# opherlieber/rltime

Measured on AMD Instinct MI355X. Metric: sampled transitions/sec (= learner steps/sec x B x T), IQN-LSTM B=512 T=80 84x84x4, higher is better.
Workload: dtype f32

## Files before the change

### include/mirl.h

```cpp
#ifndef MIRL_H
#define MIRL_H

#include <stdint.h>

#ifdef __cplusplus
extern "C" {
#endif

#define MIRL_OK 0
#define MIRL_NEED_MORE 1
#define MIRL_ERR_ARG (-1)
#define MIRL_ERR_HIP (-2)
#define MIRL_ERR_STATE (-3)
#define MIRL_ERR_NOGPU (-4)

#define MIRL_MODE_UNIFORM 0
#define MIRL_MODE_PER 1

typedef struct mirl_replay mirl_replay;

typedef struct mirl_replay_config {
  int64_t size;
  int32_t num_envs;
  int32_t env_base;
// ... 158 lines not shown
                       int32_t first, void* stream);

int mirl_frames_to_f32_nhwc(int64_t N, int32_t C, int32_t HW, const uint8_t* src, float scale,
                            float* dst, void* stream);
int mirl_frames_to_f32_nhwc_ex(int64_t N, int32_t C, int32_t HW, const uint8_t* src, float scale,
                               float* dst, int32_t per_wg, int32_t flags, void* stream);

int mirl_conv1_u8_supported(int32_t C, int32_t H, int32_t W, int32_t F, int32_t K, int32_t S);
int mirl_conv1_u8_wpk_floats(int64_t* out);
int mirl_conv1_bf16_set(int32_t mode);
int mirl_conv1_wrw_bf16_set(int32_t mode);
int mirl_conv1_u8_fwd(int64_t N, int32_t H, int32_t W, const uint8_t* x, const float* weight,
                      int64_t ws_o, int64_t ws_c, int64_t ws_h, int64_t ws_w, const float* bias,
                      float scale, float* wpk, float* y, void* stream);
int mirl_conv1_u8_fwd_ex(int64_t N, int32_t H, int32_t W, const uint8_t* x, const float* weight,
                         int64_t ws_o, int64_t ws_c, int64_t ws_h, int64_t ws_w, const float* bias,
                         float scale, float* wpk, float* y, int32_t flags, void* stream);

int mirl_conv1_u8_wrw_scratch_floats(int64_t* out);
int mirl_conv1_u8_wrw(int64_t N, int32_t H, int32_t W, const uint8_t* x, const float* g, float scale,
                      float* scratch, float* dw, int64_t ws_o, int64_t ws_c, int64_t ws_h, int64_t ws_w,
                      void* stream);
int mirl_conv1_u8_wrw_ex(int64_t N, int32_t H, int32_t W, const uint8_t* x, const float* g, float scale,
                         float* scratch, float* dw, int64_t ws_o, int64_t ws_c, int64_t ws_h, int64_t ws_w,
                         int32_t flags, void* stream);
int mirl_conv1_u8_wrw_masked(int64_t N, int32_t H, int32_t W, const uint8_t* x, const float* dy, const float* y, float scale,
                             float* scratch, float* dw, int64_t ws_o, int64_t ws_c, int64_t ws_h, int64_t ws_w,
                             float* db, void* stream);

int mirl_conv2_bwd_data_supported(int32_t C, int32_t F, int32_t K, int32_t S, int32_t IH, int32_t IW,
                                  int32_t OH, int32_t OW);
int mirl_conv2_bwd_data(int64_t N, int32_t OH, int32_t OW, const float* g, const float* weight,
                        int64_t ws_o, int64_t ws_c, int64_t ws_h, int64_t ws_w, float* wpk, float* dx,
                        void* stream);
int mirl_conv2_bwd_data_wpk_floats(int64_t* floats);
int mirl_conv2_bwd_data_ex(int64_t N, int32_t OH, int32_t OW, const float* g, const float* weight, int64_t ws_o,
                           int64_t ws_c, int64_t ws_h, int64_t ws_w, float* wpk, int64_t wpk_floats, float* dx, int32_t pipe,
                           void* stream);
int mirl_conv3_bwd_data_supported(int32_t C, int32_t F, int32_t K, int32_t S, int32_t IH, int32_t IW, int32_t OH, int32_t OW);
int mirl_conv3_bwd_data_wpk_floats(int64_t* floats);
int mirl_conv3_bwd_data(int64_t N, int32_t OH, int32_t OW, const float* g, const float* weight, int64_t ws_o,
                        int64_t ws_c, int64_t ws_h, int64_t ws_w, float* wpk, int64_t wpk_floats, float* dx, void* stream);

int mirl_gemm3_supported(int32_t layout, int64_t M, int64_t N, int64_t K);
int mirl_gemm3_workspace_bytes(int32_t layout, int64_t M, int64_t N, int64_t K, int64_t* bytes);
int mirl_gemm3(int32_t layout, int64_t M, int64_t N, int64_t K, const float* A, int64_t lda,
               const float* B, int64_t ldb, float* C, int64_t ldc, const float* bias, int32_t relu,
               void* workspace, int64_t workspace_bytes, void* stream);
int mirl_gemm3_mid_set(int32_t mode);
int mirl_gemm3_nt_mul(int64_t M, int64_t N, int64_t K, const float* A, int64_t lda, const float* B,
                      int64_t ldb, float* C, int64_t ldc, const float* bias, int32_t relu,
                      const float* mul, int64_t ldmul, int32_t group_shift, float* pre, int64_t ldpre,
                      void* stream);
int mirl_gemm3_head_workspace_bytes(int64_t M, int64_t N, int64_t* bytes);
int mirl_gemm3_nt_head(int64_t M, int64_t N, int64_t K, const float* A, int64_t lda, const float* B, int64_t ldb,
                       float* C, int64_t ldc, const float* bias, int32_t relu, const float* w2, int32_t O,
                       const float* bias2, float* out2, int64_t ldo, void* workspace, int64_t workspace_bytes, void* stream);
int mirl_gemm3_nn_qp_partial_rows(int64_t M, int64_t* rows);
int mirl_gemm3_nn_qp(int64_t M, int64_t N, int64_t K, const float* A, int64_t lda, const float* B, int64_t ldb,
                     const float* emb, int64_t ldemb, const float* x, int64_t ldx, float* d_pre, int64_t ldd,
                     float* dx, int64_t lddx, float* db_partial, void* stream);

int mirl_conv3_fwd_supported(int32_t C, int32_t F, int32_t KH, int32_t KW, int32_t S, int32_t H, int32_t W);
int mirl_conv3_fwd(int64_t N, int32_t H, int32_t W, int32_t C, int32_t F, int32_t KH, int32_t KW, int32_t S,
                   const float* x, const float* w, const float* bias, int32_t relu, float* y, void* stream);

int mirl_conv_wrw_b3_supported(int32_t C, int32_t F, int32_t KH, int32_t KW, int32_t S, int32_t H, int32_t W);
int mirl_conv_wrw_b3_scratch_bytes(int32_t C, int32_t F, int32_t KH, int32_t KW, int64_t* bytes);
int mirl_conv_wrw_b3(int64_t N, int32_t H, int32_t W, int32_t C, int32_t F, int32_t KH, int32_t KW, int32_t S,
                     const float* x, const float* g, void* scratch, int64_t scratch_bytes, float* dw, void* stream);

int mirl_bias_relu_rows(int64_t rows, int32_t C, float* y, const float* bias, void* stream);
int mirl_colsum_blocks(int64_t rows, int32_t C, int32_t* blocks);
int mirl_relu_bwd_bias_rows(int64_t rows, int32_t C, const float* dy, const float* y, float* g,
                            float* db, float* partial, int32_t blocks, void* stream);
int mirl_cos_embed(int64_t rows, int32_t D, const float* tau, const float* freq, float* phi, void* stream);
int mirl_cos_embed_rng(int64_t rows, int32_t D, uint64_t seed, const uint64_t* step, const float* freq,
                       float* phi, float* tau_out, void* stream);
int mirl_iqn_mul_fwd(int64_t M, int32_t N, int32_t C, const float* x, const float* emb, float* out, void* stream);
int mirl_iqn_mul_bwd(int64_t M, int32_t N, int32_t C, const float* g, const float* emb, const float* x,
                     float* d_pre, float* dx, float* db, float* partial, int32_t blocks, void* stream);

int mirl_dueling_tail_bwd(int64_t M, int32_t H1, int32_t Hv, int32_t A, int32_t Q, const float* ga,
                          const float* gv, const float* wo, const float* wq, const float* both,
                          float* g, float* db, float* partial, int32_t blocks, void* stream);
int mirl_dueling_tail_bwd_w(int64_t M, int32_t H1, int32_t Hv, int32_t A, int32_t Q, const float* ga,
                            const float* gv, const float* wo, const float* wq, const float* both, float* g,
                            float* db, float* partial, int32_t blocks, float* dwj, float* partial_w,
                            void* stream);

int mirl_actor_head(int32_t E, int32_t N, int32_t A, const float* adv, const float* val, int32_t Q,
                    const double* eps, const double* expo, double eps_min, const float* u, const int64_t* rnd,
                    int32_t* actions, float* qvalues, float* eps_used, void* stream);
int mirl_actor_head_rng(int32_t E, int32_t N, int32_t A, const float* adv, int32_t adv_pitch, const float* val, int32_t Q,
                        const double* eps, const double* expo, double eps_min, uint64_t rng_seed,
                        const uint64_t* rng_step, int32_t* actions, float* qvalues, float* eps_used, void* stream);
int mirl_actor_head_c51(int32_t E, int32_t A, int32_t Z, const float* adv, int32_t adv_pitch, const float* val,
                        int32_t val_pitch, const float* support, const double* eps, const double* expo, double eps_min,
                        const float* u, const int64_t* rnd, uint64_t rng_seed, const uint64_t* rng_step,
                        int32_t* actions, float* qvalues, float* eps_used, void* stream);
int mirl_stack_shift(int32_t E, int32_t P, int32_t plane_bytes, const uint8_t* in, uint8_t* out,
                     const uint8_t* newest, const uint8_t* dones, void* stream);
#define MIRL_STEP_ADVANCE (~0ull)
int mirl_actor_pre(int32_t E, int32_t H, int32_t A, const float* rewards_raw, const uint8_t* dones,
                   const int32_t* actions, const float* h, const float* c, float* xh_tail, int64_t xh_pitch,
                   float* c_in, float* state_pack, float* initials, float* rewards_out, uint8_t* dones_out,
// ... 92 lines not shown
```

### rltime_amd/_lib.py

```python
import ctypes as C
import os

import torch

_HERE = os.path.dirname(os.path.abspath(__file__))
LIB_PATH = os.path.join(_HERE, "librltime_hip.so")

MIRL_OK = 0
MIRL_NEED_MORE = 1
MODE_UNIFORM = 0
MODE_PER = 1
INT32_MIN = -2 ** 31


MIRL_OK, MIRL_ERR_ARG, MIRL_ERR_HIP, MIRL_ERR_STATE, MIRL_ERR_NOGPU = 0, -1, -2, -3, -4


class MirlError(RuntimeError):
    code = None


class ReplayConfig(C.Structure):
    _fields_ = [
        ("size", C.c_int64),
# ... 75 lines not shown

_vp, _i32, _i64, _u64, _f64 = C.c_void_p, C.c_int32, C.c_int64, C.c_uint64, C.c_double
_P = C.POINTER

_SIGNATURES = {
    "mirl_device_count": [],
    "mirl_replay_create": [_P(ReplayConfig), _P(_vp)],
    "mirl_replay_destroy": [_vp],
    "mirl_replay_ingest": [_vp, _P(Ingest), _vp],
    "mirl_replay_ingest_plan": [_vp, _i32, _i32, _vp, _vp],
    "mirl_replay_ingest_planned": [_vp, _i32, _P(Ingest), _vp],
    "mirl_ingest_fused_set": [_i32],
    "mirl_replay_prime_stack": [_vp, _vp, _i64, _vp],
    "mirl_replay_needed_feed_count": [_vp, _i32, _i32, _P(_i64)],
    "mirl_replay_sample": [_vp, _i32, _f64, _vp, _u64, _vp, _vp, _vp, _vp, _vp, _vp, _vp],
    "mirl_replay_sample_ready": [_vp, _i32, _P(_i32)],
    "mirl_replay_sample_skip": [_vp, _i32],
    "mirl_replay_tree_root": [_vp, _vp, _vp],
    "mirl_replay_sample_global": [_vp, _i32, _i32, _i32, _i32, _i32, _vp, _f64, _u64, _vp, _vp, _vp, _vp, _vp, _vp, _vp, _vp],
    "mirl_replay_profile": [_vp, _i32, _P(_i64), _P(_f64)],
    "mirl_profile_set": [_i32],
    "mirl_profile_collect": [_P(_i32)],
    "mirl_profile_get": [_i32, C.c_char_p, _i32, _P(_i64), _P(_f64), _P(_f64)],
    "mirl_profile_get_flop": [_i32, _vp],
    "mirl_profile_reset": [],
    "mirl_replay_save": [_vp, C.c_char_p],
    "mirl_replay_load": [_vp, C.c_char_p],
    "mirl_replay_uniform_total": [_vp, _P(_i64)],
    "mirl_replay_set_train_quota": [_vp, _i64],
    "mirl_replay_state_rows": [_vp, _P(_i32), _P(_i32)],
    "mirl_replay_gather": [_vp, _i32, _vp, _vp, _vp, _vp, _P(Batch), _vp],
    "mirl_replay_update_losses": [_vp, _i64, _vp, _vp, _vp],
    "mirl_replay_stats": [_vp, _P(_i64), _P(_i64), _P(_i64), _P(_i64), _P(_i64)],
    "mirl_replay_env_meta": [_vp, _vp, _vp],
    "mirl_replay_free_slots": [_vp, _vp, _P(_i64)],
    "mirl_replay_slot_table": [_vp, _vp, _vp],
    "mirl_replay_tree_nodes": [_vp, _vp, _vp, _vp],
    "mirl_replay_tree_set_leaves": [_vp, _i64, _vp, _vp, _vp],
    "mirl_replay_tree_find": [_vp, _i32, _vp, _vp, _vp],
    "mirl_replay_losses_peek": [_vp, _i32, _i64, _i32, _vp],
    "mirl_q_target_dqn": [_i64, _i32, _vp, _vp, _vp, _vp, _vp, _f64, _f64, _vp, _vp],
    "mirl_q_target_iqn": [_i64, _i32, _i32, _i32, _vp, _vp, _vp, _vp, _vp, _f64, _f64, _vp, _vp],
    "mirl_loss_dqn": [_i64, _i32, _vp, _vp, _vp, _vp, _f64, _i32, _f64, _vp, _vp, _vp, _vp],
    "mirl_loss_iqn": [_i64, _i32, _i32, _i32, _vp, _vp, _vp, _vp, _vp, _f64, _f64, _vp, _vp, _vp, _vp],
    "mirl_q_target_c51": [_i64, _i32, _i32, _vp, _vp, _vp, _vp, _vp, _vp, _f64, _f64, _f64, _f64, _i32, _vp, _vp],
    "mirl_loss_c51": [_i64, _i32, _i32, _vp, _vp, _vp, _vp, _i32, _f64, _f64, _vp, _vp, _vp, _vp],
    "mirl_actor_head_c51": [_i32, _i32, _i32, _vp, _i32, _vp, _i32, _vp, _vp, _vp, _f64, _vp, _vp, _u64, _vp, _vp, _vp, _vp, _vp],
    "mirl_lstm_cell_fwd": [_i32, _i32, _vp, _vp, _vp, _vp, _vp, _vp, _vp, _vp],
    "mirl_lstm_seq_supported": [_i32, _i32, _i32],
    "mirl_lstm_seq_workspace_bytes": [_i32, _i32, _P(_i64)],
    "mirl_lstm_seq_fwd": [_i32, _i32, _i32, _vp, _vp, _vp, _vp, _vp, _vp, _vp, _vp, _vp, _vp, _vp, _i32, _vp, _vp],
    "mirl_lstm_seq_status": [_P(_i32)],
    "mirl_gemm3_mid_set": [_i32],
    "mirl_lstm_seq_fwd_grid": [_i32, _i32, _P(_i32), _P(_i64), _P(_i32), _P(_i32)],
    "mirl_lstm_seq_bwd_supported": [_i32, _i32, _i32],
    "mirl_lstm_seq_bwd_workspace_bytes": [_i32, _i32, _P(_i64)],
    "mirl_lstm_seq_bwd": [_i32, _i32, _i32, _vp, _vp, _vp, _vp, _vp, _vp, _vp, _vp],
    "mirl_lstm_cell_bwd": [_i32, _i32, _vp, _vp, _vp, _vp, _vp, _vp, _vp, _i32, _vp],
    "mirl_frames_to_f32_nhwc": [_i64, _i32, _i32, _vp, C.c_float, _vp, _vp],
    "mirl_frames_to_f32_nhwc_ex": [_i64, _i32, _i32, _vp, C.c_float, _vp, _i32, _i32, _vp],
    "mirl_conv1_u8_supported": [_i32, _i32, _i32, _i32, _i32, _i32],
    "mirl_conv1_bf16_set": [_i32],
    "mirl_conv1_wrw_bf16_set": [_i32],
    "mirl_conv1_u8_wpk_floats": [_P(_i64)],
    "mirl_conv1_u8_fwd": [_i64, _i32, _i32, _vp, _vp, _i64, _i64, _i64, _i64, _vp, C.c_float, _vp, _vp, _vp],
    "mirl_conv1_u8_fwd_ex": [_i64, _i32, _i32, _vp, _vp, _i64, _i64, _i64, _i64, _vp, C.c_float, _vp, _vp, _i32, _vp],
    "mirl_conv1_u8_wrw_scratch_floats": [_P(_i64)],
    "mirl_conv1_u8_wrw_ex": [_i64, _i32, _i32, _vp, _vp, C.c_float, _vp, _vp, _i64, _i64, _i64, _i64, _i32, _vp],
    "mirl_conv1_u8_wrw_masked": [_i64, _i32, _i32, _vp, _vp, _vp, C.c_float, _vp, _vp, _i64, _i64, _i64, _i64, _vp, _vp],
    "mirl_conv1_u8_wrw": [_i64, _i32, _i32, _vp, _vp, C.c_float, _vp, _vp, _i64, _i64, _i64, _i64, _vp],
    "mirl_conv2_bwd_data_supported": [_i32, _i32, _i32, _i32, _i32, _i32, _i32, _i32],
    "mirl_conv2_bwd_data": [_i64, _i32, _i32, _vp, _vp, _i64, _i64, _i64, _i64, _vp, _vp, _vp],
    "mirl_conv2_bwd_data_wpk_floats": [_P(_i64)],
    "mirl_conv3_bwd_data_supported": [_i32, _i32, _i32, _i32, _i32, _i32, _i32, _i32],
    "mirl_conv3_bwd_data_wpk_floats": [_P(_i64)],
    "mirl_conv3_bwd_data": [_i64, _i32, _i32, _vp, _vp, _i64, _i64, _i64, _i64, _vp, _i64, _vp, _vp],
    "mirl_conv2_bwd_data_ex": [_i64, _i32, _i32, _vp, _vp, _i64, _i64, _i64, _i64, _vp, _i64, _vp, _i32, _vp],
    "mirl_conv3_fwd_supported": [_i32, _i32, _i32, _i32, _i32, _i32, _i32],
    "mirl_conv3_fwd": [_i64, _i32, _i32, _i32, _i32, _i32, _i32, _i32, _vp, _vp, _vp, _i32, _vp, _vp],
    "mirl_conv_wrw_b3_supported": [_i32, _i32, _i32, _i32, _i32, _i32, _i32],
    "mirl_conv_wrw_b3_scratch_bytes": [_i32, _i32, _i32, _i32, _P(_i64)],
    "mirl_conv_wrw_b3": [_i64, _i32, _i32, _i32, _i32, _i32, _i32, _i32, _vp, _vp, _vp, _i64, _vp, _vp],
    "mirl_gemm3_supported": [_i32, _i64, _i64, _i64],
    "mirl_gemm3_workspace_bytes": [_i32, _i64, _i64, _i64, _P(_i64)],
    "mirl_gemm3": [_i32, _i64, _i64, _i64, _vp, _i64, _vp, _i64, _vp, _i64, _vp, _i32, _vp, _i64, _vp],
    "mirl_gemm3_nt_mul": [_i64, _i64, _i64, _vp, _i64, _vp, _i64, _vp, _i64, _vp, _i32, _vp, _i64, _i32, _vp, _i64, _vp],
    "mirl_gemm3_nn_qp_partial_rows": [_i64, _P(_i64)],
    "mirl_gemm3_nn_qp": [_i64, _i64, _i64, _vp, _i64, _vp, _i64, _vp, _i64, _vp, _i64, _vp, _i64, _vp, _i64, _vp, _vp],
    "mirl_gemm3_head_workspace_bytes": [_i64, _i64, _P(_i64)],
    "mirl_gemm3_nt_head": [_i64, _i64, _i64, _vp, _i64, _vp, _i64, _vp, _i64, _vp, _i32, _vp, _i32, _vp, _vp, _i64, _vp, _i64, _vp],
    "mirl_act_conv_supported": [_i32, _i32, _i32, _i32, _i32, _i32, _i32],
    "mirl_act_conv_fwd": [_i32, _i64, _i32, _i32, _vp, _vp, _vp, _vp, _i64, _vp],
    "mirl_act_lstm_supported": [_i32, _i32, _i32],
    "mirl_act_lstm_workspace_bytes": [_i32, _i32, _i32, _P(_i64)],
    "mirl_act_lstm_fwd": [_i32, _i32, _i32, _vp, _i64, _vp, _vp, _vp, _vp, _vp, _vp, _vp],
    "mirl_act_embed": [_i32, _i32, _i32, _i32, _vp, _vp, _vp, _u64, _vp, _vp, _vp, _vp, _vp, _vp],
    "mirl_act_head_supported": [_i32, _i32, _i32, _i32, _i32, _i32],
    "mirl_act_head_parts": [_i32, _i32, _P(_i32), _P(_i32)],
    "mirl_act_head_hidden": [_i32, _i32, _i32, _i32, _vp, _vp, _vp, _vp, _vp, _vp],
    "mirl_act_head_select": [_i32, _i32, _i32, _i32, _i32, _vp, _vp, _i32, _vp, _vp, _f64, _u64, _vp, _vp, _vp, _vp],
    "mirl_bias_relu_rows": [_i64, _i32, _vp, _vp, _vp],
    "mirl_colsum_blocks": [_i64, _i32, _P(_i32)],
    "mirl_relu_bwd_bias_rows": [_i64, _i32, _vp, _vp, _vp, _vp, _vp, _i32, _vp],
    "mirl_cos_embed": [_i64, _i32, _vp, _vp, _vp, _vp],
    "mirl_cos_embed_rng": [_i64, _i32, _u64, _vp, _vp, _vp, _vp, _vp],
    "mirl_adam_clip_workspace_bytes": [_i32, _vp, _vp],
# ... 95 lines not shown
```

### rltime_amd/csrc/gemm3.hip

```cpp
#include "common.hpp"
#include "split3.hpp"
#include <stdlib.h>

namespace mirl {

struct G3Args {
  const float* A; const float* B; float* C; const float* bias;
  int64_t M, N, K;
  int64_t lda, ldb, ldc;
  int relu;
  int mt, nt;
  int splits;
  int steps_per_split;
  const float* mul; int64_t ldmul; int mul_shift;
  float* pre; int64_t ldpre;
  int vec_ok;
  const float* w2; float* part;
  float* gsum; int64_t ldgsum;
};


template <bool KC>
struct G3Loader {
  const float* p[2];
  int64_t step;
  int64_t ld;
  int lds_off;
  __device__ __forceinline__ void init(const float* base, int64_t ld_, int64_t row0, int64_t rows, int64_t k0, int t) {
    ld = ld_;
    if (KC) {
      const int r = t >> 2, kq = t & 3;
#pragma unroll
      for (int h = 0; h < 2; ++h) {
        int64_t row = row0 + r + 128 * h; if (row > rows - 1) row = rows - 1;
        p[h] = base + row * ld + k0 + kq * 4;
      }
      step = 16;
      lds_off = r * G3_PITCH + kq * 8;
    } else {
      const int kq = t >> 7, r = t & 127;
#pragma unroll
      for (int h = 0; h < 2; ++h) {
        int64_t row = row0 + r + 128 * h; if (row > rows - 1) row = rows - 1;
        p[h] = base + (k0 + kq * 4) * ld + row;
      }
      step = 16 * ld;
      lds_off = r * G3_PITCH + kq * 8;
    }
  }
  __device__ __forceinline__ void load(float (&v)[2][4]) {
#pragma unroll
    for (int h = 0; h < 2; ++h) {
      if (KC) {
        const float4 q = *reinterpret_cast<const float4*>(p[h]);
        v[h][0] = q.x; v[h][1] = q.y; v[h][2] = q.z; v[h][3] = q.w;
      } else {
#pragma unroll
        for (int e = 0; e < 4; ++e) v[h][e] = p[h][e * ld];
      }
      p[h] += step;
    }
  }
  __device__ __forceinline__ void store(char* planes, const float (&v)[2][4]) const {
#pragma unroll
    for (int h = 0; h < 2; ++h) {
      uint2 a, b, c;
      g3_split4(v[h], a, b, c);
      char* d = planes + lds_off + h * 128 * G3_PITCH;
      *reinterpret_cast<uint2*>(d) = a;
      *reinterpret_cast<uint2*>(d + G3_PLANE) = b;
      *reinterpret_cast<uint2*>(d + 2 * G3_PLANE) = c;
    }
  }
};

template <int TI>
__device__ __forceinline__ void g3_compute(const char* stage, g3_f32x16 (&acc)[TI][2], int a_off, int b_off) {
  const char* pa = stage + a_off;
  const char* pb = stage + 3 * G3_PLANE + b_off;
  constexpr int PA[6] = {2, 0, 1, 1, 0, 0};
  constexpr int PB[6] = {0, 2, 1, 0, 1, 0};
  g3_bf16x8 b[3][2];
#pragma unroll
  for (int p = 0; p < 3; ++p)
#pragma unroll
    for (int j = 0; j < 2; ++j) b[p][j] = *reinterpret_cast<const g3_bf16x8*>(pb + p * G3_PLANE + j * 32 * G3_PITCH);
  constexpr int IW = TI >= 2 ? 2 : 1;
#pragma unroll
  for (int ih = 0; ih < TI / IW; ++ih) {
    g3_bf16x8 a[3][IW];
#pragma unroll
    for (int p = 0; p < 3; ++p)
#pragma unroll
      for (int i = 0; i < IW; ++i) a[p][i] = *reinterpret_cast<const g3_bf16x8*>(pa + p * G3_PLANE + (ih * IW + i) * 32 * G3_PITCH);
#pragma unroll
    for (int c = 0; c < 6; ++c)
#pragma unroll
      for (int i = 0; i < IW; ++i)
#pragma unroll
        for (int j = 0; j < 2; ++j) acc[ih * IW + i][j] = g3_mfma(a[PA[c]][i], b[PB[c]][j], acc[ih * IW + i][j]);
  }
}


template <bool AKC, bool BKC, int EP, bool VEC, bool NARROW = false>
__global__ void __launch_bounds__(512)
k_gemm3(G3Args g) {
  constexpr int TI = NARROW ? 1 : 4;
  extern __shared__ __attribute__((aligned(16))) char g3_lds[];
  const int t = threadIdx.x, lane = t & 63, wave = t >> 6;
  const int b = blockIdx.x, xcd = b & 7, l = b >> 3, L = gridDim.x >> 3;
  const int64_t nk_all = g.K / 16;
  const int E = g.splits > 1 ? l + 1 : ((g.mt + 7) / 8) * g.nt;
  int split = 0;
  int64_t ks0 = 0, nk = nk_all;

  const int wu = __builtin_amdgcn_readfirstlane(wave);
  const int wm = NARROW ? 0 : (wu & 1), wn = NARROW ? 0 : (wu >> 1);
  const int row_w = NARROW ? wu * 32 : wm * 128;
  const int a_off = (row_w + (lane & 31)) * G3_PITCH + (lane >> 5) * 16;
  const int b_off = (wn * 64 + (lane & 31)) * G3_PITCH + (lane >> 5) * 16;
  const bool stage_first = (wu >> 2) & 1;

  int e = l, it = 0, jt = 0;
  if (g.splits > 1) {
    const int tiles = g.mt * g.nt, tile = l % tiles;
    split = xcd + 8 * (l / tiles);
    it = tile / g.nt; jt = tile % g.nt;
    ks0 = (int64_t)split * g.steps_per_split;
    nk = nk_all - ks0; if (nk > g.steps_per_split) nk = g.steps_per_split;
    if (nk < 0) nk = 0;
  } else {
    for (; e < E; e += L) { jt = e % g.nt; it = (e / g.nt) * 8 + xcd; if (it < g.mt) break; }
    if (e >= E) return;
  }

  G3Loader<AKC> la; G3Loader<BKC> lb;
  float va[2][4], vb[2][4];
  la.init(g.A, g.lda, (int64_t)it * 256, g.M, ks0 * 16, t);
  lb.init(g.B, g.ldb, (int64_t)jt * 256, g.N, ks0 * 16, t);
  if (nk > 0) { la.load(va); lb.load(vb); }

  g3_f32x16 acc[TI][2];
  while (true) {
    const int64_t m0 = (int64_t)it * 256, n0 = (int64_t)jt * 256;
#pragma unroll
    for (int i = 0; i < TI; ++i)
#pragma unroll
      for (int j = 0; j < 2; ++j)
#pragma unroll
        for (int r = 0; r < 16; ++r) acc[i][j][r] = 0.0f;

    if (nk > 0) {
      la.store(g3_lds, va); lb.store(g3_lds + 3 * G3_PLANE, vb);
      if (nk > 1) { la.load(va); lb.load(vb); }
    }
    g3_barrier();
    for (int64_t k = 0; k < nk; ++k) {
      const char* cur = g3_lds + (k & 1) * G3_STAGE;
      char* nxt = g3_lds + ((k + 1) & 1) * G3_STAGE;
      if (stage_first) {
        if (k + 1 < nk) { la.store(nxt, va); lb.store(nxt + 3 * G3_PLANE, vb); }
        if (k + 2 < nk) { la.load(va); lb.load(vb); }
      }
      __builtin_amdgcn_s_setprio(1);
      g3_compute<TI>(cur, acc, a_off, b_off);
      __builtin_amdgcn_s_setprio(0);
      if (!stage_first) {
        if (k + 1 < nk) { la.store(nxt, va); lb.store(nxt + 3 * G3_PLANE, vb); }
        if (k + 2 < nk) { la.load(va); lb.load(vb); }
      }
      g3_barrier();
    }

    bool more = false;
    if (g.splits <= 1) {
      for (e += L; e < E; e += L) { jt = e % g.nt; it = (e / g.nt) * 8 + xcd; if (it < g.mt) break; }
      more = e < E;
      if (more) {
        la.init(g.A, g.lda, (int64_t)it * 256, g.M, 0, t);
        lb.init(g.B, g.ldb, (int64_t)jt * 256, g.N, 0, t);
        la.load(va); lb.load(vb);
      }
    }

    float* C = g.C + (g.splits > 1 ? (int64_t)split * g.M * g.N : 0);
    if (VEC) {
      float* tl = reinterpret_cast<float*>(g3_lds) + wu * (64 * G3_EPITCH);
      constexpr int HALVES = NARROW ? 1 : 2, II = NARROW ? 1 : 2, QN = NARROW ? 8 : 16;
      float* w2l = reinterpret_cast<float*>(g3_lds) + 8 * (64 * G3_EPITCH);
      float bj[2] = {0.f, 0.f};
      g3_f32x4 sb = {0.f, 0.f, 0.f, 0.f};
      if (EP == 2) {
        const int64_t wc = n0 + (t & 63) * 4;
        float4 w = make_float4(0.f, 0.f, 0.f, 0.f);
        if (wc < g.N) w = *reinterpret_cast<const float4*>(g.w2 + (int64_t)(t >> 6) * g.N + wc);
        *reinterpret_cast<float4*>(w2l + (t >> 6) * 256 + (t & 63) * 4) = w;
#pragma unroll
        for (int j = 0; j < 2; ++j) {
          const int64_t cj = n0 + wn * 64 + j * 32 + (lane & 31);
          bj[j] = (g.bias && cj < g.N) ? g.bias[cj] : 0.f;
        }
#pragma unroll
        for (int i = 0; i < TI; ++i)
#pragma unroll
          for (int j = 0; j < 2; ++j)
#pragma unroll
            for (int r = 0; r < 16; ++r) {
              float v = acc[i][j][r] + bj[j];
              acc[i][j][r] = (g.relu && !(v > 0.f)) ? 0.f : v;
            }
        g3_barrier();
      }
#pragma unroll
      for (int h = 0; h < HALVES; ++h) {
#pragma unroll
        for (int ii = 0; ii < II; ++ii)
#pragma unroll
          for (int j = 0; j < 2; ++j)
#pragma unroll
            for (int r = 0; r < 16; ++r)
              tl[(ii * 32 + (r & 3) + 8 * (r >> 2) + 4 * (lane >> 5)) * G3_EPITCH + j * 32 + (lane & 31)] = acc[II * h + ii][j][r];
        asm volatile("s_waitcnt lgkmcnt(0)" ::: "memory");
        const int c4 = lane & 15;
        const int64_t col = n0 + wn * 64 + c4 * 4;
        float4 bv = make_float4(0.f, 0.f, 0.f, 0.f);
        if (EP != 2 && g.bias && col < g.N) {
          bv = *reinterpret_cast<const float4*>(g.bias + col);
        }
        if (EP == 2) {
          const int rg = lane & 15, cq = lane >> 4;
          const int64_t cb = (n0 >> 6) + wn;
#pragma unroll 1
          for (int ip = 0; ip < 2; ++ip) {
            float ps[2][8];
#pragma unroll
            for (int i = 0; i < 2; ++i)
#pragma unroll
              for (int o = 0; o < 8; ++o) ps[i][o] = 0.f;
#pragma unroll 1
            for (int c = 0; c < 4; ++c) {
              asm volatile("" ::: "memory");
// ... 241 lines not shown
    asm volatile("s_waitcnt lgkmcnt(0)" ::: "memory");
#pragma unroll
    for (int q = 0; q < 4; ++q) {
      const int rl = q * 8 + (lane >> 3);
      const int64_t row = m0 + wm * 128 + i * 32 + rl;
      float4 v = *reinterpret_cast<const float4*>(tl + rl * G3M_EPITCH + c4 * 4);
      if (row < g.M && col < g.N) {
        v.x += bv.x; v.y += bv.y; v.z += bv.z; v.w += bv.w;
        if (g.relu) { v.x = v.x > 0.f ? v.x : 0.f; v.y = v.y > 0.f ? v.y : 0.f; v.z = v.z > 0.f ? v.z : 0.f; v.w = v.w > 0.f ? v.w : 0.f; }
        *reinterpret_cast<float4*>(g.C + row * g.ldc + col) = v;
      }
    }
    asm volatile("s_waitcnt lgkmcnt(0)" ::: "memory");
  }
}

__global__ void __launch_bounds__(256)
k_gemm3_reduce(const float* __restrict__ partial, int splits, int64_t M, int64_t N, float* __restrict__ out, int64_t ldc) {
  const int64_t n4 = N >> 2;
  const int64_t total = M * n4;
  for (int64_t i = (int64_t)blockIdx.x * blockDim.x + threadIdx.x; i < total; i += (int64_t)gridDim.x * blockDim.x) {
    const int64_t row = i / n4, c4 = i - row * n4;
    float4 s = make_float4(0.f, 0.f, 0.f, 0.f);
    for (int k = 0; k < splits; ++k) {
      const float4 v = *reinterpret_cast<const float4*>(partial + ((int64_t)k * M + row) * N + c4 * 4);
      s.x += v.x; s.y += v.y; s.z += v.z; s.w += v.w;
    }
    *reinterpret_cast<float4*>(out + row * ldc + c4 * 4) = s;
  }
}

__global__ void __launch_bounds__(256)
k_g3_head_reduce(const float* __restrict__ part, int ncb, int64_t M, int O, const float* __restrict__ bias2,
                 float* __restrict__ out, int64_t ldo) {
  for (int64_t i = (int64_t)blockIdx.x * 256 + threadIdx.x; i < M * 2; i += (int64_t)gridDim.x * 256) {
    const int64_t row = i >> 1;
    const int half = (int)(i & 1);
    float4 sum = make_float4(0.f, 0.f, 0.f, 0.f);
    for (int cb = 0; cb < ncb; ++cb) {
      const float4 v = *reinterpret_cast<const float4*>(part + ((int64_t)cb * M + row) * 8 + half * 4);
      sum.x += v.x; sum.y += v.y; sum.z += v.z; sum.w += v.w;
    }
    const float r[4] = {sum.x, sum.y, sum.z, sum.w};
#pragma unroll
    for (int e = 0; e < 4; ++e) {
      const int o = half * 4 + e;
      if (o < O) out[row * ldo + o] = r[e] + (bias2 ? bias2[o] : 0.f);
    }
  }
}

static int g_g3_mid_mode = -1;

static int g3_splits(int64_t M, int64_t N, int64_t K) {
  const int64_t tiles = ((M + 255) / 256) * ((N + 255) / 256);
  int64_t s = 8 * ((256 + 8 * tiles - 1) / (8 * tiles));
  const int64_t nk = K / 16;
  while (s > 8 && nk / s < 64) s -= 8;
  return (int)s;
}

}

extern "C" int mirl_gemm3_supported(int32_t layout, int64_t M, int64_t N, int64_t K) {
  if (layout < 0 || layout > 2) return 0;
  if (M < 1 || N < 1 || K < 16 || (K % 16)) return 0;
  if (M >= (1LL << 31) || N >= (1LL << 31)) return 0;
  if (layout == 2) {
    if (N % 4) return 0;
    if (K / 16 < 8) return 0;
  }
  return 1;
}

extern "C" int mirl_gemm3_workspace_bytes(int32_t layout, int64_t M, int64_t N, int64_t K, int64_t* bytes) {
  using namespace mirl;
  if (!bytes) return fail(MIRL_ERR_ARG, "gemm3_workspace_bytes: null out");
  if (!mirl_gemm3_supported(layout, M, N, K)) return fail(MIRL_ERR_ARG, "gemm3: unsupported layout / shape");
  *bytes = layout == 2 ? (int64_t)g3_splits(M, N, K) * M * N * (int64_t)sizeof(float) : 0;
  return MIRL_OK;
}

namespace mirl {
struct G3Opt {
  const float* mul = nullptr; int64_t ldmul = 0; int32_t mul_shift = 0;
  float* pre = nullptr; int64_t ldpre = 0;
  const float* w2 = nullptr; float* part = nullptr;
  float* gsum = nullptr; int64_t ldgsum = 0;
};

struct G3Kernel { const void* fn; const char* name; };
static G3Kernel g3_kernel(int layout, int vec, bool mul, bool w2, bool gsum, bool narrow) {
  static const void* const plain[4][2] = {{(const void*)k_gemm3<true, true, 0, false>, (const void*)k_gemm3<true, true, 0, true>},
                                          {(const void*)k_gemm3<true, false, 0, false>, (const void*)k_gemm3<true, false, 0, true>},
                                          {nullptr , (const void*)k_gemm3<false, false, 0, true>},
                                          {(const void*)k_gemm3<true, true, 1, false>, (const void*)k_gemm3<true, true, 1, true>}};
  static const char* const names[4] = {"k_gemm3_nt", "k_gemm3_nn", "k_gemm3_tn", "k_gemm3_nt_mul"};
  if (gsum) return {(const void*)k_gemm3<true, false, 3, true>, "k_gemm3_nn_qp"};
  if (w2) return {(const void*)k_gemm3<true, true, 2, true>, "k_gemm3_nt_head"};
  if (narrow) return {(const void*)k_gemm3<false, false, 0, true, true>, "k_gemm3_tn"};
  const int which = mul ? 3 : layout;
  return {plain[which][vec], names[which]};
}
}

static int g3_launch(int32_t layout, int64_t M, int64_t N, int64_t K, const float* A, int64_t lda, const float* B,
                     int64_t ldb, float* C, int64_t ldc, const float* bias, int32_t relu, void* workspace,
                     int64_t workspace_bytes, void* stream, const mirl::G3Opt& o = mirl::G3Opt()) {
  using namespace mirl;
  if (!mirl_gemm3_supported(layout, M, N, K)) return fail(MIRL_ERR_ARG, "gemm3: unsupported layout / shape");
  if (!A || !B || (!C && !o.w2)) return fail(MIRL_ERR_ARG, "gemm3: null operand");
  const bool akc = layout != 2, bkc = layout == 0;
  if (akc && ((lda % 4) || !aligned16(A) || lda < K)) return fail(MIRL_ERR_ARG, "gemm3: A must be 16-byte aligned with lda % 4 == 0");
  if (bkc && ((ldb % 4) || !aligned16(B) || ldb < K)) return fail(MIRL_ERR_ARG, "gemm3: B must be 16-byte aligned with ldb % 4 == 0");
  if (!akc && lda < M) return fail(MIRL_ERR_ARG, "gemm3: lda < M");
  if (!bkc && ldb < N) return fail(MIRL_ERR_ARG, "gemm3: ldb < N");
  if (ldc < N) return fail(MIRL_ERR_ARG, "gemm3: ldc < N");
  if (layout == 2 && (bias || relu)) return fail(MIRL_ERR_ARG, "gemm3: no epilogue with split K");
  hipStream_t st = (hipStream_t)stream;
  G3Args g;
  g.A = A; g.B = B; g.C = C; g.bias = bias; g.M = M; g.N = N; g.K = K; g.lda = lda; g.ldb = ldb; g.ldc = ldc;
  g.relu = relu ? 1 : 0;
  g.mul = o.mul; g.ldmul = o.ldmul; g.mul_shift = o.mul_shift; g.pre = o.pre; g.ldpre = o.ldpre;
  g.w2 = o.w2; g.part = o.part; g.gsum = o.gsum; g.ldgsum = o.ldgsum;
  g.vec_ok = (N % 4 == 0) && (ldc % 4 == 0) && aligned16(C, o.w2, bias, o.mul, o.pre) && (!o.mul || o.ldmul % 4 == 0) && (!o.pre || o.ldpre % 4 == 0);
  g.mt = (int)((M + 255) / 256); g.nt = (int)((N + 255) / 256);
  g.splits = 1; g.steps_per_split = (int)(K / 16);
  unsigned grid = (unsigned)(8 * ((g.mt + 7) / 8) * g.nt);
  if (K <= 128) {
    const unsigned resident = (unsigned)(cu_count() / 8 * 8);
    if (resident && grid > resident) grid = resident;
  }
  if (layout == 2) {
    g.splits = g3_splits(M, N, K);
    const int64_t need = (int64_t)g.splits * M * N * (int64_t)sizeof(float);
    if (!workspace || workspace_bytes < need || (ldc % 4) || !aligned16(workspace, C))
      return fail(MIRL_ERR_ARG, "gemm3: split-K workspace too small / misaligned");
    g.steps_per_split = (int)((K / 16 + g.splits - 1) / g.splits);
    g.C = (float*)workspace; g.ldc = N;
    grid = (unsigned)(g.mt * g.nt * g.splits);
  }
  const int vec = g.vec_ok ? 1 : 0;
  const double flop = 2.0 * (double)M * (double)N * (double)K;
  if (g_g3_mid_mode != 0 && layout == 0 && !o.mul && !o.w2 && !o.gsum && vec && (N % 4) == 0 && (int64_t)g.mt * g.nt < 192 && N > 128 &&
      ((int64_t)g.mt * ((N + G3M_BROWS - 1) / G3M_BROWS) >= 192 || (int64_t)g.mt * g.nt < 24)) {
    if (int rc = raise_lds_limit(k_gemm3_mid, G3M_LDS)) return rc;
    g.nt = (int)((N + G3M_BROWS - 1) / G3M_BROWS);
    const unsigned mgrid = (unsigned)(8 * ((g.mt + 7) / 8) * g.nt);
    ProfScope ps("k_gemm3_nt_mid", 4.0 * ((double)M * K + (double)N * K + (double)M * N), st, flop);
    void* kargs[] = {(void*)&g};
    MIRL_HIP(hipLaunchKernel((const void*)k_gemm3_mid, dim3(mgrid), dim3(512), kargs, G3M_LDS, st));
    return MIRL_OK;
  }
  if (o.gsum) {
    if (!vec || layout != 1 || !o.mul || o.mul_shift != 5 || !o.pre || !o.part || (o.ldgsum % 4) || !aligned16(o.gsum, o.part) || (M % 32))
      return fail(MIRL_ERR_ARG, "gemm3: the fused feature-product backward needs the NN form, groups of 32 rows and 16-byte aligned rows");
  } else if (o.w2) {
    if (!vec || layout != 0 || o.mul || !o.part) return fail(MIRL_ERR_ARG, "gemm3: the fused following layer needs the NT form with 16-byte aligned rows");
  }
  const G3Kernel k = g3_kernel(layout, vec, o.mul, o.w2, o.gsum, layout == 2 && N <= 64);
  if (int rc = raise_lds_limit(k.fn, G3_LDS)) return rc;
  {
    double bytes = 4.0 * ((double)M * K + (double)N * K + (double)M * N * (layout == 2 ? (double)g.splits : 1.0));
    if (o.mul) bytes += 4.0 * ((o.pre ? (double)M * N : 0.0) + (double)(M >> o.mul_shift) * N * (o.gsum ? 2.0 : 1.0));
    if (o.w2) bytes += 4.0 * (8.0 * (double)N + 8.0 * (double)M * (double)((N + 63) / 64)) - (C ? 0.0 : 4.0 * (double)M * N);
    ProfScope ps(k.name, bytes, st, flop);
    void* kargs[] = {(void*)&g};
    MIRL_HIP(hipLaunchKernel(k.fn, dim3(grid), dim3(512), kargs, G3_LDS, st));
  }
  if (layout == 2) {
    ProfScope ps("k_gemm3_reduce", (double)(g.splits + 1) * (double)M * (double)N * 4.0, st);
    hipLaunchKernelGGL(k_gemm3_reduce, dim3(capped_grid((M * (N / 4) + 255) / 256, 4096)), dim3(256), 0, st, (const float*)workspace, g.splits, M, N, C, ldc);
    MIRL_LAUNCH_CHECK();
  }
  return MIRL_OK;
}

extern "C" int mirl_gemm3(int32_t layout, int64_t M, int64_t N, int64_t K, const float* A, int64_t lda, const float* B,
                          int64_t ldb, float* C, int64_t ldc, const float* bias, int32_t relu, void* workspace,
                          int64_t workspace_bytes, void* stream) {
  return g3_launch(layout, M, N, K, A, lda, B, ldb, C, ldc, bias, relu, workspace, workspace_bytes, stream);
}

extern "C" int mirl_gemm3_mid_set(int32_t mode) {
  if (mode < -1 || mode > 1) return mirl::fail(MIRL_ERR_ARG, "gemm3_mid_set: mode is -1 (default), 0 or 1");
  mirl::g_g3_mid_mode = mode;
  return MIRL_OK;
}

extern "C" int mirl_gemm3_nt_mul(int64_t M, int64_t N, int64_t K, const float* A, int64_t lda, const float* B, int64_t ldb,
                                 float* C, int64_t ldc, const float* bias, int32_t relu, const float* mul, int64_t ldmul,
                                 int32_t group_shift, float* pre, int64_t ldpre, void* stream) {
  using namespace mirl;
  if (!mul || group_shift < 0 || group_shift > 30 || ldmul < N || (pre && ldpre < N))
    return fail(MIRL_ERR_ARG, "gemm3_nt_mul: bad multiplier / pre-activation arguments");
  G3Opt o;
  o.mul = mul; o.ldmul = ldmul; o.mul_shift = group_shift; o.pre = pre; o.ldpre = ldpre;
  return g3_launch(0, M, N, K, A, lda, B, ldb, C, ldc, bias, relu, nullptr, 0, stream, o);
}

extern "C" int mirl_gemm3_nn_qp_partial_rows(int64_t M, int64_t* rows) {
  if (!rows || M < 1) return mirl::fail(MIRL_ERR_ARG, "gemm3_nn_qp_partial_rows: M >= 1");
  *rows = 2 * ((M + 255) / 256);
  return MIRL_OK;
}

extern "C" int mirl_gemm3_nn_qp(int64_t M, int64_t N, int64_t K, const float* A, int64_t lda, const float* B, int64_t ldb,
                                const float* emb, int64_t ldemb, const float* x, int64_t ldx, float* d_pre, int64_t ldd,
                                float* dx, int64_t lddx, float* db_partial, void* stream) {
  using namespace mirl;
  if (!emb || !x || !d_pre || !dx || !db_partial || ldemb < N || ldx < N || lddx < N || (ldemb % 4) || !aligned16(emb))
    return fail(MIRL_ERR_ARG, "gemm3_nn_qp: bad embedding / feature / output arguments");
  G3Opt o;
  o.mul = x; o.ldmul = ldx; o.mul_shift = 5; o.pre = const_cast<float*>(emb); o.ldpre = ldemb;
  o.part = db_partial; o.gsum = dx; o.ldgsum = lddx;
  return g3_launch(1, M, N, K, A, lda, B, ldb, d_pre, ldd, nullptr, 0, nullptr, 0, stream, o);
}

extern "C" int mirl_gemm3_head_workspace_bytes(int64_t M, int64_t N, int64_t* bytes) {
  if (!bytes || M < 1 || N < 1) return mirl::fail(MIRL_ERR_ARG, "bad gemm3_head_workspace_bytes arguments");
  *bytes = 8 * (int64_t)sizeof(float) * M * ((N + 255) / 256 * 4);
  return MIRL_OK;
}

extern "C" int mirl_gemm3_nt_head(int64_t M, int64_t N, int64_t K, const float* A, int64_t lda, const float* B, int64_t ldb,
                                  float* C, int64_t ldc, const float* bias, int32_t relu, const float* w2, int32_t O,
                                  const float* bias2, float* out2, int64_t ldo, void* workspace, int64_t workspace_bytes,
                                  void* stream) {
  using namespace mirl;
  int64_t need = 0;
  if (O < 1 || O > 8 || !w2 || !out2 || ldo < O || !workspace || mirl_gemm3_head_workspace_bytes(M, N, &need) || workspace_bytes < need ||
      !aligned16(workspace) || (N % 4))
    return fail(MIRL_ERR_ARG, "bad gemm3_nt_head arguments (1 <= O <= 8, N % 4 == 0, 16-byte aligned workspace of head_workspace_bytes)");
  if (!C) ldc = N;
  G3Opt o;
  o.w2 = w2; o.part = (float*)workspace;
  if (int rc = g3_launch(0, M, N, K, A, lda, B, ldb, C, ldc, bias, relu, nullptr, 0, stream, o)) return rc;
  const int ncb = (int)((N + 255) / 256 * 4);
  hipStream_t st = (hipStream_t)stream;
// ... 6 lines not shown
```

Baseline: 484,500.

## Split GEMM into body, sub-tiled tail wave, and narrow column strip launches

Adds a planner that uses the CU count to spot a poorly filled final wave of 256x256 tiles. It then re-launches that remainder as 128- or 64-row sub-tiles, and sends a leftover column strip of 64 or fewer columns to the narrow kernel. The kernel's work enumeration becomes a unit range (e0..e1 with a row offset) so that several launches can cover disjoint parts of the output. This targets wave-quantisation idle time, at the cost of extra launches and less efficient small tiles.

Result: no change. 488,100 (median of 6 runs) (+0.7%).

```diff
diff --git a/include/mirl.h b/include/mirl.h
--- a/include/mirl.h
+++ b/include/mirl.h
@@ -234,6 +234,8 @@
                       int64_t ldb, float* C, int64_t ldc, const float* bias, int32_t relu,
                       const float* mul, int64_t ldmul, int32_t group_shift, float* pre, int64_t ldpre,
                       void* stream);
+int mirl_gemm3_tail_set(int32_t mode, int32_t pretend_cus);
+int mirl_gemm3_plan_describe(int32_t layout, int64_t M, int64_t N, int64_t K, int32_t* out);
 int mirl_gemm3_head_workspace_bytes(int64_t M, int64_t N, int64_t* bytes);
 int mirl_gemm3_nt_head(int64_t M, int64_t N, int64_t K, const float* A, int64_t lda, const float* B, int64_t ldb,
                        float* C, int64_t ldc, const float* bias, int32_t relu, const float* w2, int32_t O,
diff --git a/rltime_amd/_lib.py b/rltime_amd/_lib.py
--- a/rltime_amd/_lib.py
+++ b/rltime_amd/_lib.py
@@ -151,6 +151,8 @@
     "mirl_lstm_seq_fwd": [_i32, _i32, _i32, _vp, _vp, _vp, _vp, _vp, _vp, _vp, _vp, _vp, _vp, _vp, _i32, _vp, _vp],
     "mirl_lstm_seq_status": [_P(_i32)],
     "mirl_gemm3_mid_set": [_i32],
+    "mirl_gemm3_tail_set": [_i32, _i32],
+    "mirl_gemm3_plan_describe": [_i32, _i64, _i64, _i64, _P(_i32)],
     "mirl_lstm_seq_fwd_grid": [_i32, _i32, _P(_i32), _P(_i64), _P(_i32), _P(_i32)],
     "mirl_lstm_seq_bwd_supported": [_i32, _i32, _i32],
     "mirl_lstm_seq_bwd_workspace_bytes": [_i32, _i32, _P(_i64)],
diff --git a/rltime_amd/csrc/gemm3.hip b/rltime_amd/csrc/gemm3.hip
--- a/rltime_amd/csrc/gemm3.hip
+++ b/rltime_amd/csrc/gemm3.hip
@@ -1,5 +1,6 @@
 #include "common.hpp"
 #include "split3.hpp"
+#include "gemm3_plan.hpp"
 #include <stdlib.h>
 
 namespace mirl {
@@ -12,6 +13,8 @@
   int mt, nt;
   int splits;
   int steps_per_split;
+  int e0, e1;
+  int64_t csplit;
   const float* mul; int64_t ldmul; int mul_shift;
   float* pre; int64_t ldpre;
   int vec_ok;
@@ -20,9 +23,9 @@
 };
 
 
-template <bool KC>
+template <bool KC, int H = 2>
 struct G3Loader {
-  const float* p[2];
+  const float* p[H];
   int64_t step;
   int64_t ld;
   int lds_off;
@@ -31,7 +34,7 @@
     if (KC) {
       const int r = t >> 2, kq = t & 3;
 #pragma unroll
-      for (int h = 0; h < 2; ++h) {
+      for (int h = 0; h < H; ++h) {
         int64_t row = row0 + r + 128 * h; if (row > rows - 1) row = rows - 1;
         p[h] = base + row * ld + k0 + kq * 4;
       }
@@ -40,7 +43,7 @@
     } else {
       const int kq = t >> 7, r = t & 127;
 #pragma unroll
-      for (int h = 0; h < 2; ++h) {
+      for (int h = 0; h < H; ++h) {
         int64_t row = row0 + r + 128 * h; if (row > rows - 1) row = rows - 1;
         p[h] = base + (k0 + kq * 4) * ld + row;
       }
@@ -48,9 +51,9 @@
       lds_off = r * G3_PITCH + kq * 8;
     }
   }
-  __device__ __forceinline__ void load(float (&v)[2][4]) {
-#pragma unroll
-    for (int h = 0; h < 2; ++h) {
+  __device__ __forceinline__ void load(float (&v)[H][4]) {
+#pragma unroll
+    for (int h = 0; h < H; ++h) {
       if (KC) {
         const float4 q = *reinterpret_cast<const float4*>(p[h]);
         v[h][0] = q.x; v[h][1] = q.y; v[h][2] = q.z; v[h][3] = q.w;
@@ -61,9 +64,9 @@
       p[h] += step;
     }
   }
-  __device__ __forceinline__ void store(char* planes, const float (&v)[2][4]) const {
-#pragma unroll
-    for (int h = 0; h < 2; ++h) {
+  __device__ __forceinline__ void store(char* planes, const float (&v)[H][4]) const {
+#pragma unroll
+    for (int h = 0; h < H; ++h) {
       uint2 a, b, c;
       g3_split4(v[h], a, b, c);
       char* d = planes + lds_off + h * 128 * G3_PITCH;
@@ -103,47 +106,51 @@
 }
 
 
-template <bool AKC, bool BKC, int EP, bool VEC, bool NARROW = false>
+template <bool AKC, bool BKC, int EP, bool VEC, bool NARROW = false, int ROWS = 256>
 __global__ void __launch_bounds__(512)
 k_gemm3(G3Args g) {
-  constexpr int TI = NARROW ? 1 : 4;
+  static_assert(ROWS == 256 || (!NARROW && EP == 0 && (ROWS == 128 || ROWS == 64)), "sub-tiles: plain form, 128 or 64 rows");
+  constexpr int TI = NARROW ? 1 : ROWS / 64;
+  constexpr int HA = ROWS == 256 ? 2 : 1;
   extern __shared__ __attribute__((aligned(16))) char g3_lds[];
   const int t = threadIdx.x, lane = t & 63, wave = t >> 6;
   const int b = blockIdx.x, xcd = b & 7, l = b >> 3, L = gridDim.x >> 3;
   const int64_t nk_all = g.K / 16;
-  const int E = g.splits > 1 ? l + 1 : ((g.mt + 7) / 8) * g.nt;
+  const int U = (g.e1 - g.e0) * (256 / ROWS);
   int split = 0;
   int64_t ks0 = 0, nk = nk_all;
 
   const int wu = __builtin_amdgcn_readfirstlane(wave);
   const int wm = NARROW ? 0 : (wu & 1), wn = NARROW ? 0 : (wu >> 1);
-  const int row_w = NARROW ? wu * 32 : wm * 128;
+  const int row_w = NARROW ? wu * 32 : wm * (TI * 32);
   const int a_off = (row_w + (lane & 31)) * G3_PITCH + (lane >> 5) * 16;
   const int b_off = (wn * 64 + (lane & 31)) * G3_PITCH + (lane >> 5) * 16;
   const bool stage_first = (wu >> 2) & 1;
 
-  int e = l, it = 0, jt = 0;
+  int u = l, e = 0, ro = 0, it = 0, jt = 0;
+  auto find = [&]() {
+    for (; u < U; u += L) {
+      g3_unit(g.e0, ROWS, u, e, ro);
+      if (g3_list_entry(g.mt, g.nt, g.splits, e, xcd, it, jt, split) && (int64_t)it * 256 + ro < g.M) return true;
+    }
+    return false;
+  };
+  if (!find()) return;
   if (g.splits > 1) {
-    const int tiles = g.mt * g.nt, tile = l % tiles;
-    split = xcd + 8 * (l / tiles);
-    it = tile / g.nt; jt = tile % g.nt;
     ks0 = (int64_t)split * g.steps_per_split;
     nk = nk_all - ks0; if (nk > g.steps_per_split) nk = g.steps_per_split;
     if (nk < 0) nk = 0;
-  } else {
-    for (; e < E; e += L) { jt = e % g.nt; it = (e / g.nt) * 8 + xcd; if (it < g.mt) break; }
-    if (e >= E) return;
-  }
-
-  G3Loader<AKC> la; G3Loader<BKC> lb;
-  float va[2][4], vb[2][4];
-  la.init(g.A, g.lda, (int64_t)it * 256, g.M, ks0 * 16, t);
+  }
+
+  G3Loader<AKC, HA> la; G3Loader<BKC> lb;
+  float va[HA][4], vb[2][4];
+  la.init(g.A, g.lda, (int64_t)it * 256 + ro, g.M, ks0 * 16, t);
   lb.init(g.B, g.ldb, (int64_t)jt * 256, g.N, ks0 * 16, t);
   if (nk > 0) { la.load(va); lb.load(vb); }
 
   g3_f32x16 acc[TI][2];
   while (true) {
-    const int64_t m0 = (int64_t)it * 256, n0 = (int64_t)jt * 256;
+    const int64_t m0 = (int64_t)it * 256 + ro, n0 = (int64_t)jt * 256;
 #pragma unroll
     for (int i = 0; i < TI; ++i)
 #pragma unroll
@@ -175,19 +182,19 @@
 
     bool more = false;
     if (g.splits <= 1) {
-      for (e += L; e < E; e += L) { jt = e % g.nt; it = (e / g.nt) * 8 + xcd; if (it < g.mt) break; }
-      more = e < E;
+      u += L;
+      more = find();
       if (more) {
-        la.init(g.A, g.lda, (int64_t)it * 256, g.M, 0, t);
+        la.init(g.A, g.lda, (int64_t)it * 256 + ro, g.M, 0, t);
         lb.init(g.B, g.ldb, (int64_t)jt * 256, g.N, 0, t);
         la.load(va); lb.load(vb);
       }
     }
 
-    float* C = g.C + (g.splits > 1 ? (int64_t)split * g.M * g.N : 0);
+    float* C = g.C + (g.splits > 1 ? (int64_t)split * g.csplit : 0);
     if (VEC) {
       float* tl = reinterpret_cast<float*>(g3_lds) + wu * (64 * G3_EPITCH);
-      constexpr int HALVES = NARROW ? 1 : 2, II = NARROW ? 1 : 2, QN = NARROW ? 8 : 16;
+      constexpr int HALVES = TI == 4 ? 2 : 1, II = TI >= 2 ? 2 : 1, QN = 8 * II;
       float* w2l = reinterpret_cast<float*>(g3_lds) + 8 * (64 * G3_EPITCH);
       float bj[2] = {0.f, 0.f};
       g3_f32x4 sb = {0.f, 0.f, 0.f, 0.f};
@@ -535,12 +542,12 @@
 
 static int g_g3_mid_mode = -1;
 
-static int g3_splits(int64_t M, int64_t N, int64_t K) {
-  const int64_t tiles = ((M + 255) / 256) * ((N + 255) / 256);
-  int64_t s = 8 * ((256 + 8 * tiles - 1) / (8 * tiles));
-  const int64_t nk = K / 16;
-  while (s > 8 && nk / s < 64) s -= 8;
-  return (int)s;
+static int g_g3_tail_mode = -1;
+static int g_g3_tail_cus = 0;
+
+static G3Plan g3_current_plan(int layout, int64_t M, int64_t N, int64_t K) {
+  if (g_g3_tail_mode == 1) return g3_plan(layout, M, N, K, g_g3_tail_cus, true);
+  return g3_plan(layout, M, N, K, g_g3_tail_mode == 0 ? 0 : cu_count(), false);
 }
 
 }
@@ -584,6 +591,13 @@
   if (narrow) return {(const void*)k_gemm3<false, false, 0, true, true>, "k_gemm3_tn"};
   const int which = mul ? 3 : layout;
   return {plain[which][vec], names[which]};
+}
+static const void* g3_plan_kernel(int layout, int rows) {
+  static const void* const fns[3][3] = {
+      {(const void*)k_gemm3<true, true, 0, true, true>, (const void*)k_gemm3<true, true, 0, true, false, 128>, (const void*)k_gemm3<true, true, 0, true, false, 64>},
+      {(const void*)k_gemm3<true, false, 0, true, true>, (const void*)k_gemm3<true, false, 0, true, false, 128>, (const void*)k_gemm3<true, false, 0, true, false, 64>},
+      {(const void*)k_gemm3<false, false, 0, true, true>, (const void*)k_gemm3<false, false, 0, true, false, 128>, (const void*)k_gemm3<false, false, 0, true, false, 64>}};
+  return fns[layout][rows == 0 ? 0 : rows == 128 ? 1 : 2];
 }
 }
 
@@ -608,7 +622,8 @@
   g.w2 = o.w2; g.part = o.part; g.gsum = o.gsum; g.ldgsum = o.ldgsum;
   g.vec_ok = (N % 4 == 0) && (ldc % 4 == 0) && aligned16(C, o.w2, bias, o.mul, o.pre) && (!o.mul || o.ldmul % 4 == 0) && (!o.pre || o.ldpre % 4 == 0);
   g.mt = (int)((M + 255) / 256); g.nt = (int)((N + 255) / 256);
-  g.splits = 1; g.steps_per_split = (int)(K / 16);
+  g.splits = 1; g.steps_per_split = (int)(K / 16); g.csplit = 0;
+  g.e0 = 0; g.e1 = ((g.mt + 7) / 8) * g.nt;
   unsigned grid = (unsigned)(8 * ((g.mt + 7) / 8) * g.nt);
   if (K <= 128) {
     const unsigned resident = (unsigned)(cu_count() / 8 * 8);
@@ -620,12 +635,15 @@
     if (!workspace || workspace_bytes < need || (ldc % 4) || !aligned16(workspace, C))
       return fail(MIRL_ERR_ARG, "gemm3: split-K workspace too small / misaligned");
     g.steps_per_split = (int)((K / 16 + g.splits - 1) / g.splits);
-    g.C = (float*)workspace; g.ldc = N;
+    g.C = (float*)workspace; g.ldc = N; g.csplit = M * N;
+    g.e1 = g.mt * g.nt * (g.splits / 8);
     grid = (unsigned)(g.mt * g.nt * g.splits);
   }
   const int vec = g.vec_ok ? 1 : 0;
   const double flop = 2.0 * (double)M * (double)N * (double)K;
-  if (g_g3_mid_mode != 0 && layout == 0 && !o.mul && !o.w2 && !o.gsum && vec && (N % 4) == 0 && (int64_t)g.mt * g.nt < 192 && N > 128 &&
+  G3Plan plan = g3_current_plan(layout, M, N, K);
+  if (o.mul || o.w2 || o.gsum || !vec || (layout == 2 && N <= 64)) plan.single = 1;
+  if (g_g3_mid_mode != 0 && plan.single && layout == 0 && !o.mul && !o.w2 && !o.gsum && vec && (N % 4) == 0 && (int64_t)g.mt * g.nt < 192 && N > 128 &&
       ((int64_t)g.mt * ((N + G3M_BROWS - 1) / G3M_BROWS) >= 192 || (int64_t)g.mt * g.nt < 24)) {
     if (int rc = raise_lds_limit(k_gemm3_mid, G3M_LDS)) return rc;
     g.nt = (int)((N + G3M_BROWS - 1) / G3M_BROWS);
@@ -648,8 +666,25 @@
     if (o.mul) bytes += 4.0 * ((o.pre ? (double)M * N : 0.0) + (double)(M >> o.mul_shift) * N * (o.gsum ? 2.0 : 1.0));
     if (o.w2) bytes += 4.0 * (8.0 * (double)N + 8.0 * (double)M * (double)((N + 63) / 64)) - (C ? 0.0 : 4.0 * (double)M * N);
     ProfScope ps(k.name, bytes, st, flop);
-    void* kargs[] = {(void*)&g};
-    MIRL_HIP(hipLaunchKernel(k.fn, dim3(grid), dim3(512), kargs, G3_LDS, st));
+    if (plan.single) {
+      void* kargs[] = {(void*)&g};
+      MIRL_HIP(hipLaunchKernel(k.fn, dim3(grid), dim3(512), kargs, G3_LDS, st));
+    } else {
+      G3Launch ls[3];
+      const int nl = g3_plan_launches(plan, N, ls);
+      for (int i = 0; i < nl; ++i) {
+        const G3Launch& l = ls[i];
+        G3Args a = g;
+        a.B = B + (bkc ? l.col_off * ldb : l.col_off); a.C = g.C + l.col_off; a.bias = bias ? bias + l.col_off : nullptr;
+        a.N = l.n; a.nt = l.nt; a.e0 = l.e0; a.e1 = l.e1;
+        unsigned lgrid = (unsigned)(8 * l.units);
+        if (l.rows == 256 && K <= 128) { const unsigned resident = (unsigned)(cu_count() / 8 * 8); if (resident && lgrid > resident) lgrid = resident; }
+        const void* fn = l.rows == 256 ? k.fn : g3_plan_kernel(layout, l.rows);
+        if (int rc = raise_lds_limit(fn, G3_LDS)) return rc;
+        void* kargs[] = {(void*)&a};
+        MIRL_HIP(hipLaunchKernel(fn, dim3(lgrid), dim3(512), kargs, G3_LDS, st));
+      }
+    }
   }
   if (layout == 2) {
     ProfScope ps("k_gemm3_reduce", (double)(g.splits + 1) * (double)M * (double)N * 4.0, st);
@@ -668,6 +703,33 @@
 extern "C" int mirl_gemm3_mid_set(int32_t mode) {
   if (mode < -1 || mode > 1) return mirl::fail(MIRL_ERR_ARG, "gemm3_mid_set: mode is -1 (default), 0 or 1");
   mirl::g_g3_mid_mode = mode;
+  return MIRL_OK;
+}
+
+extern "C" int mirl_gemm3_tail_set(int32_t mode, int32_t pretend_cus) {
+  if (mode < -1 || mode > 1 || (mode == 1 && pretend_cus < 8)) return mirl::fail(MIRL_ERR_ARG, "gemm3_tail_set: mode is -1 (default), 0 or 1 with pretend_cus >= 8");
+  mirl::g_g3_tail_mode = mode;
+  mirl::g_g3_tail_cus = mode == 1 ? pretend_cus : 0;
+  return MIRL_OK;
+}
+
+extern "C" int mirl_gemm3_plan_describe(int32_t layout, int64_t M, int64_t N, int64_t K, int32_t* out) {
+  using namespace mirl;
+  if (!out) return fail(MIRL_ERR_ARG, "gemm3_plan_describe: null out");
+  if (!mirl_gemm3_supported(layout, M, N, K)) return fail(MIRL_ERR_ARG, "gemm3: unsupported layout / shape");
+  G3Plan p = g3_current_plan(layout, M, N, K);
+  if ((N % 4) || (layout == 2 && N <= 64)) p = g3_plan(layout, M, N, K, 0, false);
+  G3Launch ls[3];
+  const int nl = g3_plan_launches(p, N, ls);
+  for (int i = 0; i < 6; ++i) out[i] = 0;
+  out[0] = nl;
+  for (int i = 0; i < nl; ++i) {
+    if (ls[i].rows == 256) out[1] = 8 * ls[i].units;
+    else if (ls[i].rows) { out[2] = 256 / ls[i].rows; out[3] = 8 * ls[i].units; }
+    else { out[4] = (int32_t)ls[i].n; out[5] = 8 * ls[i].units; }
+  }
+  out[6] = p.splits;
+  out[7] = p.steps_per_split;
   return MIRL_OK;
 }
 
diff --git a/rltime_amd/csrc/gemm3_plan.hpp b/rltime_amd/csrc/gemm3_plan.hpp
--- /dev/null
+++ b/rltime_amd/csrc/gemm3_plan.hpp
@@ -0,0 +1,114 @@
+#pragma once
+#include <stdint.h>
+
+#if defined(__HIPCC__)
+#define G3P_HD __host__ __device__
+#else
+#define G3P_HD
+#endif
+
+namespace mirl {
+
+constexpr int G3_XCDS = 8;
+
+inline int g3_splits(int64_t M, int64_t N, int64_t K) {
+  const int64_t tiles = ((M + 255) / 256) * ((N + 255) / 256);
+  int64_t s = 8 * ((256 + 8 * tiles - 1) / (8 * tiles));
+  const int64_t nk = K / 16;
+  while (s > 8 && nk / s < 64) s -= 8;
+  return (int)s;
+}
+
+G3P_HD inline bool g3_list_entry(int mt, int nt, int splits, int e, int xcd, int& it, int& jt, int& split) {
+  if (splits > 1) {
+    const int tiles = mt * nt, tile = e % tiles;
+    split = xcd + G3_XCDS * (e / tiles);
+    it = tile / nt; jt = tile % nt;
+    return true;
+  }
+  split = 0;
+  jt = e % nt; it = (e / nt) * G3_XCDS + xcd;
+  return it < mt;
+}
+
+G3P_HD inline void g3_unit(int e0, int rows, int u, int& e, int& row_off) {
+  const int cut = 256 / rows;
+  e = e0 + u / cut;
+  row_off = (u % cut) * rows;
+}
+
+struct G3Plan {
+  int single;
+  int mt, nt;
+  int splits, steps_per_split;
+  int nt_body;
+  int strip_cols;
+  int strip_list;
+  int list;
+  int body_end;
+  int tail_cut;
+};
+
+inline int g3_list_len(int layout, int mt, int nt, int splits) {
+  return layout == 2 ? mt * nt * (splits / G3_XCDS) : ((mt + G3_XCDS - 1) / G3_XCDS) * nt;
+}
+
+inline double g3_tail_cost(int rem, int cpx, int cut) {
+  const double per_item = cut == 1 ? 1.0 : cut == 2 ? 0.6 : 0.4;
+  const int rounds = (rem * cut + cpx - 1) / cpx;
+  return rounds * per_item;
+}
+
+inline G3Plan g3_plan(int layout, int64_t M, int64_t N, int64_t K, int cus, bool force) {
+  G3Plan p;
+  p.mt = (int)((M + 255) / 256); p.nt = (int)((N + 255) / 256);
+  p.splits = 1; p.steps_per_split = (int)(K / 16);
+  if (layout == 2) {
+    p.splits = g3_splits(M, N, K);
+    p.steps_per_split = (int)((K / 16 + p.splits - 1) / p.splits);
+  }
+  p.single = 1; p.nt_body = p.nt; p.strip_cols = 0; p.strip_list = 0; p.tail_cut = 0;
+  p.list = g3_list_len(layout, p.mt, p.nt, p.splits);
+  p.body_end = p.list;
+  const int cpx = cus / G3_XCDS;
+  if (cpx < 1 || (!force && K <= 128)) return p;
+
+  int nt_body = p.nt, strip_cols = 0;
+  const int r = (int)(N % 256);
+  if (r > 0 && r <= 64 && p.nt > 1) { nt_body = p.nt - 1; strip_cols = r; }
+  const int list = g3_list_len(layout, p.mt, nt_body, p.splits);
+  if (!force && list < 2 * cpx) return p;
+
+  int cut = 0;
+  const int rem = list % cpx;
+  if (rem > 0 && rem * 10 <= cpx * 6) {
+    double best = g3_tail_cost(rem, cpx, 1);
+    for (int c = 2; c <= 4; c *= 2) {
+      if (rem * c > cpx) continue;
+      const double cost = g3_tail_cost(rem, cpx, c);
+      if (cost < best) { best = cost; cut = c; }
+    }
+  }
+  if (!strip_cols && !cut) return p;
+  p.single = 0;
+  p.nt_body = nt_body; p.strip_cols = strip_cols;
+  p.strip_list = strip_cols ? g3_list_len(layout, p.mt, 1, p.splits) : 0;
+  p.list = list;
+  p.tail_cut = cut;
+  p.body_end = cut ? list - rem : list;
+  return p;
+}
+
+struct G3Launch { int rows, e0, e1, nt; int64_t n, col_off; int units; };
+
+inline int g3_plan_launches(const G3Plan& p, int64_t N, G3Launch (&out)[3]) {
+  int c = 0;
+  if (p.single) { out[c++] = G3Launch{256, 0, p.list, p.nt, N, 0, p.list}; return c; }
+  const int64_t body_n = p.strip_cols ? (int64_t)p.nt_body * 256 : N;
+  if (p.body_end > 0) out[c++] = G3Launch{256, 0, p.body_end, p.nt_body, body_n, 0, p.body_end};
+  if (p.tail_cut) out[c++] = G3Launch{256 / p.tail_cut, p.body_end, p.list, p.nt_body, body_n, 0, (p.list - p.body_end) * p.tail_cut};
+  if (p.strip_cols) out[c++] = G3Launch{0, 0, p.strip_list, 1, p.strip_cols, body_n, p.strip_list};
+  return c;
+}
+
+}
```
